# twosigma/Cook

Measured on AMD Instinct MI355X. Metric: match-cycles/sec at 1M pending x 50k offers, higher is better.
Workload: dtype f64

## Files before the change

cook_amd/csrc/classfit_asm.hpp:

```cpp
#pragma once
#if CF_SLOTS_N == 12
#define CF_O_CTRL "13728"
#define CF_O_CTRL4 "13732"
#define CF_O_ARR "15280"
#define CF_O_CLS32 "9504"
#define CF_SLOT_SHIFT "9"
#define CF_SLOT_N "12"
#define CF_ROW_END "3072"
#elif CF_SLOTS_N == 24
#define CF_O_CTRL "16800"
#define CF_O_CTRL4 "16804"
#define CF_O_ARR "18352"
#define CF_O_CLS32 "12576"
#define CF_SLOT_SHIFT "10"
#define CF_SLOT_N "24"
#define CF_ROW_END "6144"
#else
#error "CF_SLOTS_N: 12 or 24"
#endif
#ifndef CF_ASM_WAIT_READS
#define CF_ASM_WAIT_READS "30"
#endif
#ifdef CF_DELAY_D
#define CF_ASM_DELAY_D "s_sleep 6\n\t"
#else
#define CF_ASM_DELAY_D
#endif
#define CF_ASM_DECIDER_RUN \
   \
  "v_lshl_add_u32 v114, v65, 3, s56\n\t" \
  "ds_read_b64 v[114:115], v114\n\t" \
  "s_ff1_i32_b64 s44, s[42:43]\n\t" \
  "s_lshl_b32 s45, s44, 12\n\t" \
  "s_add_u32 s45, s45, s59\n\t" \
  "s_lshl_b32 s47, s57, 8\n\t" \
  "s_or_b32 s47, s47, s44\n\t" \
  "s_mov_b32 s41, 1\n\t"  \
   \
  "0:\n\t" \
  "v_readlane_b32 s60, v80, s44\n\t" \
  "v_readlane_b32 s61, v81, s44\n\t" \
  "v_readlane_b32 s62, v82, s44\n\t" \
  "s_and_b32 s63, s62, 0xffff00ff\n\t"  \
  "s_cmp_lg_u32 s63, 0\n\t" \
  "s_cbranch_scc1 9f\n\t" \
                                                                                           \
  "v_mov_b32_e32 v88, s47\n\t"                                                                                                          \
  "v_add_u32_e32 v100, s46, v83\n\t"                                                                                                    \
  "s_mov_b64 exec, 1\n\t"                                                                                                               \
  "ds_write_b32 v87, v88 offset:" CF_O_CTRL4 "\n\t"                                                                                              \
  "s_mov_b64 exec, -1\n\t"                                                                                                              \
  "s_mov_b32 s82, " CF_ASM_WAIT_READS "\n\t"              \
  "1:\n\t"                                                                                                                              \
  "ds_read_b32 v92, v100\n\t"                                                                                                           \
  "ds_read_b64 v[94:95], v100 offset:8\n\t"                                                                                             \
  "ds_read_b128 v[96:99], v100 offset:16\n\t"                                                                                           \
  "ds_read_b32 v93, v100\n\t"                                                                                                           \
                                        \
  "v_subrev_u32_e32 v101, s60, v71\n\t"                                                                                                 \
  "v_subrev_u32_e32 v102, s61, v72\n\t"                                                                                                 \
  "v_cvt_f64_u32_e32 v[104:105], v101\n\t"                                                                                              \
  "v_cvt_f64_u32_e32 v[106:107], v102\n\t"                                                                                              \
  "v_mul_f64 v[104:105], v[104:105], v[66:67]\n\t"                                                                                      \
  "v_mul_f64 v[106:107], v[106:107], v[68:69]\n\t"                                                                                      \
  "v_add_f64 v[104:105], v[104:105], v[106:107]\n\t"                                                                                    \
  "v_add_f64 v[104:105], -v[104:105], 1.0\n\t"                                                                                          \
  "v_cmp_le_u32_e64 s[64:65], s60, v71\n\t"                                                                                             \
  "v_cmp_le_u32_e64 s[66:67], s61, v72\n\t"                                                                                             \
  "v_cmp_ne_u32_e64 s[68:69], 0, v64\n\t"                                                                                               \
  "s_and_b64 s[64:65], s[64:65], s[66:67]\n\t"                                                                                          \
  "s_and_b64 s[64:65], s[64:65], s[68:69]\n\t"                                                                                          \
  "s_waitcnt lgkmcnt(0)\n\t"                                                                                                            \
        \
  "s_bfe_u32 s63, s62, 0x4000c\n\t"                                                                                                     \
  "s_cmp_eq_u32 s63, 0\n\t"                                                                                                             \
  "s_cbranch_scc1 3f\n\t"                                                                                                               \
  "v_readlane_b32 s66, v85, s44\n\t"                                                                                                    \
  "v_readlane_b32 s67, v86, s44\n\t"                                                                                                    \
  "s_cmp_lt_u32 s63, 1\n\t"                                                                                                           \
  "s_cbranch_scc1 3f\n\t"                                                                                                               \
  "s_bfe_u32 s72, s66, 0x100000\n\t"                                                                      \
  "s_lshr_b32 s73, s72, 8\n\t"                                                                                                          \
  "s_lshl_b32 s73, s73, 3\n\t"                                                                                                          \
  "s_and_b32 s72, s72, 0xff\n\t"                                                                                                        \
  "v_lshrrev_b64 v[108:109], s73, v[114:115]\n\t"                                                                                       \
  "v_and_b32_e32 v108, 0xff, v108\n\t"                                                                                                  \
  "v_cmp_eq_u32_e64 s[74:75], s72, v108\n\t"                                                                                            \
  "s_and_b64 s[64:65], s[64:65], s[74:75]\n\t"                                                                                          \
  "s_cmp_lt_u32 s63, 2\n\t"                                                                                                           \
  "s_cbranch_scc1 3f\n\t"                                                                                                               \
  "s_bfe_u32 s72, s66, 0x100010\n\t"                                                                      \
  "s_lshr_b32 s73, s72, 8\n\t"                                                                                                          \
  "s_lshl_b32 s73, s73, 3\n\t"                                                                                                          \
  "s_and_b32 s72, s72, 0xff\n\t"                                                                                                        \
  "v_lshrrev_b64 v[108:109], s73, v[114:115]\n\t"                                                                                       \
  "v_and_b32_e32 v108, 0xff, v108\n\t"                                                                                                  \
  "v_cmp_eq_u32_e64 s[74:75], s72, v108\n\t"                                                                                            \
  "s_and_b64 s[64:65], s[64:65], s[74:75]\n\t"                                                                                          \
  "s_cmp_lt_u32 s63, 3\n\t"                                                                                                           \
  "s_cbranch_scc1 3f\n\t"                                                                                                               \
  "s_bfe_u32 s72, s67, 0x100000\n\t"                                                                      \
  "s_lshr_b32 s73, s72, 8\n\t"                                                                                                          \
  "s_lshl_b32 s73, s73, 3\n\t"                                                                                                          \
  "s_and_b32 s72, s72, 0xff\n\t"                                                                                                        \
  "v_lshrrev_b64 v[108:109], s73, v[114:115]\n\t"                                                                                       \
  "v_and_b32_e32 v108, 0xff, v108\n\t"                                                                                                  \
  "v_cmp_eq_u32_e64 s[74:75], s72, v108\n\t"                                                                                            \
  "s_and_b64 s[64:65], s[64:65], s[74:75]\n\t"                                                                                          \
  "s_cmp_lt_u32 s63, 4\n\t"                                                                                                           \
  "s_cbranch_scc1 3f\n\t"                                                                                                               \
  "s_bfe_u32 s72, s67, 0x100010\n\t"                                                                      \
  "s_lshr_b32 s73, s72, 8\n\t"                                                                                                          \
  "s_lshl_b32 s73, s73, 3\n\t"                                                                                                          \
  "s_and_b32 s72, s72, 0xff\n\t"                                                                                                        \
  "v_lshrrev_b64 v[108:109], s73, v[114:115]\n\t"                                                                                       \
  "v_and_b32_e32 v108, 0xff, v108\n\t"                                                                                                  \
  "v_cmp_eq_u32_e64 s[74:75], s72, v108\n\t"                                                                                            \
  "s_and_b64 s[64:65], s[64:65], s[74:75]\n\t"                                                                                          \
  "3:\n\t"                                                                                                                              \
   \
  "v_and_b32_e32 v108, 0xffffff00, v92\n\t"                                                                                             \
  "v_cmp_eq_u32_e64 s[70:71], s45, v108\n\t"                                                                                            \
  "v_cmp_eq_u32_e64 s[72:73], v92, v93\n\t"                                                                                             \
  "v_sub_u32_e32 v108, v73, v92\n\t"                                                                                                    \
  "v_and_b32_e32 v108, 0xff, v108\n\t"                                                                                                  \
  "v_cmp_gt_u32_e64 s[74:75], 3, v108\n\t"                                                                                              \
  "v_and_b32_e32 v109, 0xffff, v94\n\t"                                                                                                 \
  "v_cmp_ne_u32_e64 s[76:77], v109, v74\n\t"                                                                                            \
  "v_cmp_ne_u32_e64 s[78:79], v109, v75\n\t"                                                                                            \
  "v_cmp_gt_i32_e64 s[80:81], 0, v95\n\t"                                                                                               \
  "s_and_b64 s[74:75], s[74:75], s[76:77]\n\t"                                                                                          \
  "s_and_b64 s[74:75], s[74:75], s[78:79]\n\t"                                                                                          \
  "s_or_b64 s[74:75], s[74:75], s[80:81]\n\t"                                                                                           \
  "s_and_b64 s[72:73], s[70:71], s[72:73]\n\t"                                          \
  "s_and_b64 s[70:71], s[72:73], s[74:75]\n\t"                                                                                            \
  "s_andn2_b64 s[76:77], s[52:53], s[70:71]\n\t"                                                                     \
  "s_cmp_eq_u64 s[76:77], 0\n\t"                                                                                                          \
  "s_cbranch_scc1 2f\n\t"                                                                                                                 \
   \
   \
  "s_and_b64 s[78:79], s[76:77], s[72:73]\n\t"                                                                                            \
  "s_cmp_eq_u64 s[78:79], 0\n\t"                                                                                                          \
  "s_cbranch_scc1 4f\n\t"                                                                                                                 \
  "v_and_b32_e32 v109, 0x3fff, v95\n\t"                                                                                                   \
  "s_and_b64 s[72:73], s[64:65], s[54:55]\n\t"                                                   \
  "10:\n\t"                                                                                                                               \
  "s_ff1_i32_b64 s83, s[78:79]\n\t"                                                                                                       \
  "v_readlane_b32 s63, v109, s83\n\t"                                                                                                     \
  "s_bitset0_b64 s[78:79], s83\n\t"                                                                                                       \
  "v_cmp_eq_u32_e64 vcc, s63, v65\n\t"                                                                                                    \
  "s_and_b64 vcc, vcc, s[72:73]\n\t"                                                                                                      \
  "s_cmp_eq_u64 vcc, 0\n\t"                                                                                                               \
  "s_cbranch_scc1 11f\n\t"                                                                                                                \
  "s_bitset1_b64 s[80:81], s83\n\t"                                                                                                       \
  "s_bitset0_b64 s[76:77], s83\n\t"                                                                                                       \
  "11:\n\t"                                                                                                                               \
  "s_cmp_lg_u64 s[78:79], 0\n\t"                                                                                                          \
  "s_cbranch_scc1 10b\n\t"                                                                                                                \
  "s_cmp_eq_u64 s[76:77], 0\n\t"                                                                                                          \
  "s_cbranch_scc1 2f\n\t"                                                                                                                 \
  "4:\n\t"                                                                                                                                \
  "s_sub_u32 s82, s82, 1\n\t"      \
  "s_cmp_eq_u32 s82, 0\n\t"                                                                                                             \
  "s_cbranch_scc1 9f\n\t"                                                                                                               \
  "s_sleep 1\n\t"                                                                                                                       \
  "s_branch 1b\n\t"                                                                                                                     \
  "2:\n\t"                                                                                                                              \
  "s_andn2_b64 s[74:75], s[52:53], s[80:81]\n\t"                                                                        \
  "s_or_b64 s[64:65], s[64:65], s[74:75]\n\t"                                                          \
  "v_cndmask_b32_e64 v110, v98, v104, s[54:55]\n\t"                                                                                     \
  "v_cndmask_b32_e64 v111, v99, v105, s[54:55]\n\t"                                                                                     \
  "v_cndmask_b32_e64 v110, 0, v110, s[64:65]\n\t"                                                                                       \
  "v_cndmask_b32_e64 v111, 0, v111, s[64:65]\n\t"                                                                                       \
  "v_cvt_f32_f64_e32 v112, v[110:111]\n\t" \
   \
   \
   \
  "s_mov_b64 s[84:85], s[42:43]\n\t" \
  "v_mov_b32_e32 v113, v112\n\t" \
  "s_bitset0_b64 s[84:85], s44\n\t" \
  "s_add_u32 s46, s46, 256\n\t" \
  "v_max_f32_dpp v113, v113, v113 quad_perm:[1,0,3,2] row_mask:0xf bank_mask:0xf\n\t" \
  "s_ff1_i32_b64 s86, s[84:85]\n\t" \
  "s_add_u32 s62, s57, 1\n\t" \
  "v_max_f32_dpp v113, v113, v113 quad_perm:[2,3,0,1] row_mask:0xf bank_mask:0xf\n\t" \
  "s_cmp_eq_u32 s46, " CF_ROW_END "\n\t" \
  "s_cselect_b32 s46, 0, s46\n\t" \
  "v_max_f32_dpp v113, v113, v113 row_half_mirror row_mask:0xf bank_mask:0xf\n\t" \
  "s_lshl_b32 s62, s62, 8\n\t" \
  "s_or_b32 s47, s62, s86\n\t" \
  "v_max_f32_dpp v113, v113, v113 row_mirror row_mask:0xf bank_mask:0xf\n\t" \
  "s_lshl_b32 s63, s86, 12\n\t" \
  "s_add_u32 s45, s59, s63\n\t" \
  "v_max_f32_dpp v113, v113, v113 row_bcast:15 row_mask:0xa bank_mask:0xf\n\t" \
  "v_add_f32_e32 v108, 0x35000000, v112\n\t" \
  "v_and_b32_e32 v109, 0x40000000, v95\n\t" \
  "v_max_f32_dpp v113, v113, v113 row_bcast:31 row_mask:0xc bank_mask:0xf\n\t" \
  "v_cmp_ne_u32_e64 s[70:71], 0, v109\n\t" \
  "s_nop 0\n\t" \
  "v_readlane_b32 s63, v113, 63\n\t" \
  "s_cmp_eq_u32 s63, 0\n\t" \
  "s_cbranch_scc1 8f\n\t"  \
  "v_cmp_eq_f32_e64 s[78:79], s63, v112\n\t" \
  "v_cmp_le_f32_e64 s[76:77], s63, v108\n\t"  \
  "s_and_b64 s[76:77], s[76:77], s[64:65]\n\t"                                      \
  "s_bcnt1_i32_b64 s62, s[76:77]\n\t"                                                                                                   \
  "s_cmp_gt_u32 s62, 1\n\t"                                                                                                             \
  "s_cbranch_scc1 9f\n\t"                                                                                                               \
  "s_and_b64 s[70:71], s[70:71], s[76:77]\n\t"                                                                                          \
  "s_and_b64 s[70:71], s[70:71], s[74:75]\n\t"                       \
  "s_cmp_lg_u64 s[70:71], 0\n\t"                                                                                                        \
  "s_cbranch_scc1 9f\n\t"                                                                                                               \
  "s_ff1_i32_b64 s82, s[78:79]\n\t"                                                                                                     \
  "s_cmp_lt_u32 s82, 58\n\t"                                                                                                            \
  "s_cbranch_scc0 5f\n\t"                                                                                                               \
                                                                                                         \
  "v_readlane_b32 s64, v71, s82\n\t"                                                                                                    \
  "v_readlane_b32 s65, v72, s82\n\t"                                                                                                    \
  "v_readlane_b32 s66, v65, s82\n\t"                                                                                                    \
  "s_sub_u32 s67, s64, s60\n\t"                                                                                                         \
  "s_sub_u32 s70, s65, s61\n\t"                                                                                                         \
  "v_cmp_eq_u32_e64 vcc, s82, v84\n\t"                                                                                                  \
  "v_mov_b32_e32 v88, s67\n\t"                                                                                                          \
  "v_mov_b32_e32 v89, s70\n\t"                                                                                                          \
  "s_cmp_lt_u32 s67, s49\n\t" \
  "s_cselect_b32 s71, 1, 0\n\t" \
  "s_cmp_lt_u32 s70, s50\n\t" \
  "s_cselect_b32 s71, 1, s71\n\t" \
  "v_cndmask_b32_e32 v71, v71, v88, vcc\n\t"                                                                                            \
  "v_cndmask_b32_e32 v72, v72, v89, vcc\n\t"                                                                                            \
  "s_cmp_lg_u32 s71, 0\n\t"                                                                                                             \
  "s_cselect_b64 s[62:63], vcc, 0\n\t"                             \
  "s_mov_b32 s72, s44\n\t"                                                                                                              \
  "s_mov_b32 s73, 0\n\t"                                                                                                                \
  "v_cndmask_b32_e64 v64, v64, 0, s[62:63]\n\t"                                                                                         \
  "s_branch 7f\n\t"                                                                                                                     \
        \
  "5:\n\t"                                                                                                                              \
  "v_readlane_b32 s64, v96, s82\n\t"                                                                                                    \
  "v_readlane_b32 s65, v97, s82\n\t"                                                                                                    \
  "v_readlane_b32 s76, v95, s82\n\t"                                                                                                    \
  "v_readlane_b32 s77, v94, s82\n\t"                                                                                                    \
  "v_readlane_b32 s78, v73, s82\n\t"                                                                                                    \
  "s_sub_u32 s67, s64, s60\n\t"                                                                                                         \
  "s_sub_u32 s70, s65, s61\n\t"                                                                                                         \
  "s_and_b32 s66, s76, 0x3fff\n\t"                                                                                                      \
  "s_bfe_u32 s79, s76, 0x80010\n\t"                                                                                                     \
  "s_and_b32 s73, s77, 0xffff\n\t"                                                                                                      \
  "s_lshr_b32 s81, s77, 16\n\t"                                                                                                         \
  "s_sub_u32 s80, s82, 57\n\t"                                                                                                          \
  "s_cmp_lt_u32 s67, s49\n\t" \
  "s_cselect_b32 s71, 1, 0\n\t" \
  "s_cmp_lt_u32 s70, s50\n\t" \
  "s_cselect_b32 s71, 1, s71\n\t" \
  "s_bcnt1_i32_b64 s62, s[68:69]\n\t"                                                                                                   \
  "s_cmp_lg_u32 s71, 0\n\t"                                                                                                             \
  "s_cbranch_scc1 6f\n\t"                                                                                                               \
  "s_cmp_ge_u32 s62, " CF_ASM_EPOCH_LIVE "\n\t"                                                                                          \
  "s_cbranch_scc1 9f\n\t"                                  \
  "6:\n\t"                                                                                                                              \
  "s_lshl_b32 s62, s73, 3\n\t" \
  "s_lshl_b32 s63, s80, 2\n\t" \
  "s_add_u32 s78, s78, 1\n\t" \
  "v_mov_b32_e32 v88, 0\n\t" \
  "v_mov_b32_e32 v89, 0\n\t" \
  "v_add_u32_e32 v90, s62, v87\n\t" \
  "v_add_u32_e32 v91, s63, v87\n\t" \
  "v_mov_b32_e32 v100, s78\n\t"                                                                                                         \
  "s_mov_b64 exec, 1\n\t"                                                                                                               \
  "ds_write_b64 v90, v[88:89] offset:" CF_O_ARR "\n\t"                                                                                         \
  "ds_write_b32 v91, v100 offset:" CF_O_CTRL4 "\n\t"                                                                                             \
  "s_mov_b64 exec, -1\n\t"                                                                                                              \
  "v_cmp_eq_u32_e64 vcc, s82, v84\n\t"                                                                                                  \
  "v_mov_b32_e32 v101, s73\n\t" \
  "s_lshl_b32 s62, s80, 8\n\t" \
  "v_cndmask_b32_e32 v75, v75, v74, vcc\n\t" \
  "v_cndmask_b32_e32 v74, v74, v101, vcc\n\t" \
  "v_cndmask_b32_e32 v73, v73, v100, vcc\n\t" \
  "s_lshl_b32 s63, s81, 12\n\t"                                                                                                         \
  "s_or_b32 s72, s44, s62\n\t"                                                                                                          \
  "s_or_b32 s72, s72, s63\n\t"                                                                                                          \
  "s_cmp_lg_u32 s71, 0\n\t"                                                                                                             \
  "s_cbranch_scc1 7f\n\t"                                                                              \
  "s_mul_i32 s62, s79, 56\n\t" \
  "v_add_u32_e32 v90, s62, v87\n\t" \
  "ds_read_b128 v[116:119], v90 offset:" CF_O_CLS32 "\n\t"  \
  "v_mov_b32_e32 v88, s66\n\t" \
  "v_lshl_add_u32 v102, v88, 3, s56\n\t"   \
  "ds_read_b64 v[102:103], v102\n\t"                                                                                        \
  "s_andn2_b64 s[62:63], s[54:55], s[68:69]\n\t"                                                                                        \
  "s_ff1_i32_b64 s83, s[62:63]\n\t"                                                                                                     \
  "v_cmp_eq_u32_e64 vcc, s83, v84\n\t"                                                                                                  \
  "v_mov_b32_e32 v89, s79\n\t"                                                                                                          \
  "v_mov_b32_e32 v91, s67\n\t"                                                                                                          \
  "v_mov_b32_e32 v101, s70\n\t"                                                                                                         \
  "v_cndmask_b32_e64 v64, v64, 1, vcc\n\t"                                                                                              \
  "v_cndmask_b32_e32 v65, v65, v88, vcc\n\t"                                                                                            \
  "v_cndmask_b32_e32 v70, v70, v89, vcc\n\t"                                                                                            \
  "v_cndmask_b32_e32 v71, v71, v91, vcc\n\t"                                                                                            \
  "v_cndmask_b32_e32 v72, v72, v101, vcc\n\t"                                                                                           \
  "s_waitcnt lgkmcnt(0)\n\t"                                                                                                            \
  "v_cndmask_b32_e32 v66, v66, v116, vcc\n\t"                                                                                           \
  "v_cndmask_b32_e32 v67, v67, v117, vcc\n\t"                                                                                           \
  "v_cndmask_b32_e32 v68, v68, v118, vcc\n\t"                                                                                           \
  "v_cndmask_b32_e32 v69, v69, v119, vcc\n\t"  \
  "v_cndmask_b32_e32 v114, v114, v102, vcc\n\t" \
  "v_cndmask_b32_e32 v115, v115, v103, vcc\n\t"                                                                                           \
   \
  "7:\n\t"                                                                                                                              \
  "v_cmp_eq_u32_e64 vcc, s44, v84\n\t"                                                                                                  \
  "v_mov_b32_e32 v88, s66\n\t"                                                                                                          \
  "v_cmp_lt_u32_e64 s[62:63], s67, v80\n\t"                                                                                             \
  "v_cmp_lt_u32_e64 s[76:77], s70, v81\n\t"                                                                                             \
  "v_cndmask_b32_e32 v76, v76, v88, vcc\n\t"                                                                                            \
  "s_or_b64 s[62:63], s[62:63], s[76:77]\n\t"                                                                                           \
  "s_lshl_b64 s[76:77], -2, s44\n\t"                                                                                                    \
  "s_and_b64 s[62:63], s[62:63], s[76:77]\n\t"                                                                                          \
  "s_or_b64 s[38:39], s[38:39], s[62:63]\n\t"                                                                                           \
  "s_min_u32 s37, s37, s67\n\t"                                                                                                         \
  "s_min_u32 s40, s40, s70\n\t"                                                                                                         \
  "s_add_u32 s36, s36, 1\n\t"                                                                                                           \
  "v_mov_b32_e32 v88, s72\n\t"                                                                                                          \
  "v_mov_b32_e32 v89, s73\n\t"                                                                                                          \
  "v_mov_b32_e32 v90, s64\n\t"                                                                                                          \
  "v_mov_b32_e32 v91, s65\n\t" \
  "s_mov_b64 exec, 1\n\t" \
  "ds_write_b128 v77, v[88:91]\n\t" \
  "s_mov_b64 exec, -1\n\t" \
  "v_add_u32_e32 v77, 32, v77\n\t"  \
   \
  "8:\n\t" \
  CF_ASM_DELAY_D \
  "s_mov_b64 s[42:43], s[84:85]\n\t" \
  "s_mov_b32 s44, s86\n\t" \
  "s_add_u32 s57, s57, 1\n\t" \
  "s_cmp_lg_u64 s[42:43], 0\n\t" \
  "s_cbranch_scc1 0b\n\t" \
  "s_mov_b32 s41, 0\n\t" \
  "9:\n\t" \
  "s_waitcnt lgkmcnt(0)\n\t"

#define CF_ASM_CLASS_STEP                                                                                                               \
  "v_mov_b32_e32 v80, s44\n\t"                                                                                                          \
  "s_lshl_b32 s60, s45, 2\n\t"                                                                                                          \
  "s_add_u32 s60, s60, s44\n\t"                                                                                                         \
  "v_mov_b32_e32 v81, s60\n\t"                                                                                                          \
  "ds_read_b64 v[82:83], v80 offset:" CF_O_CTRL "\n\t"                                                                     \
  "ds_read_b32 v84, v81 offset:" CF_O_CTRL4 "\n\t"                                                                   \
  "s_mov_b32 s41, 3\n\t"                                                                                                                \
  "s_waitcnt lgkmcnt(0)\n\t"                                                                                                            \
  "v_readfirstlane_b32 s61, v82\n\t"                                                                                                    \
  "v_readfirstlane_b32 s42, v83\n\t"                                                                                                    \
  "v_readfirstlane_b32 s43, v84\n\t"                                                                                                    \
  "s_cmp_lg_u32 s61, 0\n\t"                                                                                                             \
  "s_cbranch_scc1 9f\n\t"                                                                                                               \
  "s_cmp_lg_u32 s43, s40\n\t"                                                                                                           \
  "s_cbranch_scc1 9f\n\t"                                                                                                               \
  "s_mov_b32 s41, 2\n\t"                                                                                                                \
                                                                                                 \
  "1:\n\t"                                                                                                                              \
  "s_cmp_eq_u64 s[36:37], 0\n\t"                                                                                                        \
  "s_cbranch_scc1 9f\n\t"                                                                                                               \
  "s_cmp_eq_u32 s39, s56\n\t"                                                                                                           \
  "s_cbranch_scc1 2f\n\t"                                                                                                               \
  "s_add_u32 s62, s36, -1\n\t"                                                                                                          \
  "s_addc_u32 s63, s37, -1\n\t"                                                                                                         \
  "s_and_b64 s[36:37], s[36:37], s[62:63]\n\t"                                                                                          \
  "s_add_u32 s38, s38, 1\n\t"                                                                                                           \
  "s_add_u32 s39, s39, 1\n\t"                                                                                                           \
  "s_cmp_eq_u32 s39, s57\n\t"                                                                                                           \
  "s_cselect_b32 s39, 0, s39\n\t"                                                                                                       \
  "s_branch 1b\n\t"                                                                                                                     \
  "2:\n\t"                                                                                                                                \
  "s_lshr_b32 s60, s42, 8\n\t"                                                                                                            \
  "s_cmp_lt_u32 s38, s60\n\t"                                          \
  "s_cbranch_scc0 12f\n\t"                                                                                                                \
  "s_mov_b32 s41, 3\n\t"                                                                                                                  \
  "s_branch 9f\n\t"                                                                                                                       \
  "12:\n\t"                                                                                                                               \
  "s_add_u32 s60, s60, s59\n\t"                                                                                                         \
  "s_cmp_ge_u32 s38, s60\n\t"                                                                                                           \
  "s_cbranch_scc1 9f\n\t"                                                                             \
  "s_ff1_i32_b64 s64, s[36:37]\n\t"                                                                                                     \
  "v_readlane_b32 s65, v72, s64\n\t"                                                                                                    \
  "v_readlane_b32 s66, v73, s64\n\t"                                                                                                    \
  "v_readlane_b32 s67, v74, s64\n\t"                                                                                                    \
  "s_mov_b32 s41, 1\n\t"                                                                                                                \
  "s_lshr_b32 s60, s67, 12\n\t"                                                                                                         \
  "s_cmp_lg_u32 s60, 0\n\t"                                                                                                             \
  "s_cbranch_scc1 9f\n\t"                                                                                \
  "s_and_b32 s60, s67, 0xff\n\t"                                                                                                        \
  "s_cmp_lg_u32 s60, s58\n\t"                                                                                                           \
  "s_cbranch_scc1 8f\n\t"                                                                                \
                                           \
  "s_bfe_u32 s60, s67, 0x30008\n\t"                                                                                                     \
  "s_bitcmp1_b32 s60, 0\n\t"                                                                                                            \
  "s_cselect_b64 vcc, -1, 0\n\t"                                                                                                        \
  "v_cndmask_b32_e32 v80, v64, v65, vcc\n\t"                                                                                            \
  "v_cndmask_b32_e32 v81, v66, v67, vcc\n\t"                                                                                            \
  "v_cndmask_b32_e32 v82, v68, v69, vcc\n\t"                                                                                            \
  "v_cndmask_b32_e32 v83, v70, v71, vcc\n\t"                                                                                            \
  "s_bitcmp1_b32 s60, 1\n\t"                                                                                                            \
  "s_cselect_b64 vcc, -1, 0\n\t"                                                                                                        \
  "v_cndmask_b32_e32 v80, v80, v81, vcc\n\t"                                                                                            \
  "v_cndmask_b32_e32 v82, v82, v83, vcc\n\t"                                                                                            \
  "s_bitcmp1_b32 s60, 2\n\t"                                                                                                            \
  "s_cselect_b64 vcc, -1, 0\n\t"                                                                                                        \
  "v_cndmask_b32_e32 v80, v80, v82, vcc\n\t"                                                                                            \
                                                                 \
  "s_mul_i32 s68, s38, 43\n\t"                                                                                                          \
  "s_lshr_b32 s68, s68, " CF_SLOT_SHIFT "\n\t"                                                                                                          \
  "s_mul_i32 s68, s68, " CF_SLOT_N "\n\t"                                                                                                          \
// ... 84 lines not shown
```

cook_amd/csrc/classfit_host.hpp:

```cpp

static int classfit_env() {
  static const int v = [] {
    const char* s = std::getenv("COOK_CLASSFIT");
    return s && (s[0] == '0' || s[0] == '1') ? s[0] - '0' : -1;
  }();
  return v;
}
static bool classfit_by_default(const cook_engine* e) {
  const int f = classfit_env();
  if (f >= 0) return f == 1;
  return g_engines_on_device[e->device & 63].load() >= 6;
}
static size_t cf_lds_bytes_host(unsigned NP, unsigned M, bool eq, unsigned G, unsigned S) {
  size_t n = sizeof(CfFixed) + (size_t)NP * 10u;
  n = (n + 7u) & ~(size_t)7u;
  if (eq) n += (size_t)M * 8u;
  n += ((size_t)G + 1u) * 2u + (size_t)G * 2u + (size_t)S * 2u;
  return n + 64u;
}
bool cf_setup(cook_engine* e, const MatchIn& in, const MatchIn* in_dev, const MatchState& st, const JobRec* jr, const JobCons* jcons, const OfferA* oa, const OfferB* ob,
              CfPoolCtx& ctx) {
  const unsigned K = in.K, M = in.M, G = in.G;
  e->cf_inelig = 0x10000u;
  if (K == 0 || M == 0 || M > CF_SORT_N || G > CF_MAXG || in.good_enough < 1.0 || in.has_x || in.reserved_bits || in.host_dup) return false;
  if (e->cf_max_host == 0xFFFFFFFFu || (size_t)e->cf_max_host > 8u * (size_t)M + 65536u) return false;
  CfBuf b{};
  b.ctl = e->cf_ctl.ensure(1);
  b.jr = jr, b.jcons = jcons, b.oa = oa, b.ob = ob;
  b.attr8 = e->cf_attr8.ensure(M);
  b.max_host = e->cf_max_host;
  b.h2o = e->cf_h2o.ensure((size_t)b.max_host + 1u);
  b.pos_fc = e->cf_pos[0].ensure(M), b.pos_fm = e->cf_pos[1].ensure(M), b.pos_cid = e->cf_pos[2].ensure(M);
  b.scr_fc = e->cf_scr[0].ensure(M), b.scr_fm = e->cf_scr[1].ensure(M), b.scr_cid = e->cf_scr[2].ensure(M);
  b.jobs = e->cf_jobs.ensure(K);
  b.gcount = e->cf_gcount.ensure(std::max(1u, G));
  b.gmem = e->cf_gmem.ensure((size_t)std::max(1u, G) * CF_GMEM);
  static_assert(sizeof(CfCtl) % 4 == 0, "cf_init clears the control block word by word");
  KM<cf_init, 256>(e, "cf_init", std::min(div_up(b.max_host + 1u, 1024u), 512u), b, b.max_host + 1u, std::max(1u, G));
  KM<cf_scan, 256>(e, "cf_scan", div_up(std::max(K, M), 256), in_dev, b, K, M);
  KM<cf_prepare, 1024>(e, "cf_prepare", 1u, in_dev, b, st.jmin, K, M, G, in.host_dup, in.reserved_bits ? 1u : 0u);
  KM<cf_pack_jobs, 256>(e, "cf_pack_jobs", div_up(K, 256), in_dev, b, K);
  static_assert(offsetof(CfCtl, t) <= 512, "the control block's head is read back through the 512-byte scratch");
  pinned_copy(e, e->h_scratch, b.ctl, offsetof(CfCtl, t), hipMemcpyDeviceToHost);
  sync(e);
  CfCtl hc;
  std::memcpy((void*)&hc, e->h_scratch, offsetof(CfCtl, t));
  e->cf_inelig = hc.inelig;
  if (hc.inelig) return false;
  const unsigned NP = (M + 63u) & ~63u;
  const unsigned S = hc.any_group ? e->cf_group_run_total + hc.n_grouped : 0u;
  if (cf_lds_bytes_host(NP, M, hc.any_eq != 0u, hc.any_group ? G : 0u, S) > CF_LDS_BYTES || S > 60000u) {
    e->cf_inelig = CF_X_SHAPE;
    return false;
  }
  ctx.in = in_dev;
  ctx.st = st;
  ctx.b = b;
  return true;
}
static void cf_prof_print(const uint32_t* q) {
#ifdef CF_PROF
  std::fprintf(stderr, "CFPROF (x16 shader cycles) decider: slow steps %u (candidates %u evaluation %u commit %u) plain steps %u in %u walk-total %u | class wave 1: poll %u answer %u answers %u idle %u idles %u | class wave 2: poll %u answer %u answers %u idle %u idles %u | walk ticks(100MHz) %u | batch boundaries: decider %u, batches without a walked job %u\n", q[27], q[24], q[25], q[26], q[28], q[29], q[31], q[32], q[33], q[35], q[36], q[37], q[40], q[41], q[43], q[44], q[45], q[CFS_TICKS_WALK], q[30], q[38]);
  std::fprintf(stderr, "CFPROF plain steps %u, C++ steps %u; steps that left the plain form: gpu kind %u, novel hosts %u, group %u, answer missing after the re-reads %u, guard band %u, epoch end %u\n", q[46], q[47], q[34] & 65535u, q[34] >> 16, q[39] & 65535u, q[39] >> 16, q[42] & 65535u, q[42] >> 16);
#else
  (void)q;
#endif
}
void cf_run(cook_engine* lead, cook_engine* const* es, unsigned n, hipStream_t stream) {
  cook_engine* e = lead;
  for (unsigned i0 = 0; i0 < n; i0 += (unsigned)CF_PACK) {
    const unsigned c = std::min<unsigned>(CF_PACK, n - i0);
    CfPack pk{};
    for (unsigned x = 0; x < (unsigned)CF_PACK; ++x) pk.c[x] = es[i0 + (x < c ? x : 0u)]->placement.walk;
    KLS("cf_walk", stream, cf_walk, c, CF_THREADS, pk);
  }
  for (unsigned i = 0; i < n; ++i) {
    const CfPoolCtx& c = es[i]->placement.walk;
    const unsigned G = es[i]->last_in.G;
    if (G) KLS("cf_group_chains", stream, cf_group_chains, div_up(G, 256), 256, c.b, c.st, G);
  }
  constexpr size_t SLOT = 16 + 48 * 4;
  if (!lead->h_cf) COOK_HIP(hipHostMalloc((void**)&lead->h_cf, 64 * SLOT, hipHostMallocDefault));
  for (unsigned i = 0; i < n; ++i) {
    char* slot = lead->h_cf + i * SLOT;
    COOK_HIP(hipMemcpyAsync(slot, es[i]->placement.walk.st.summary, 16, hipMemcpyDeviceToHost, stream));
    COOK_HIP(hipMemcpyAsync(slot + 16, es[i]->placement.walk.b.ctl->stats, 48 * 4, hipMemcpyDeviceToHost, stream));
  }
  COOK_HIP(hipStreamSynchronize(stream));
  for (unsigned i = 0; i < n; ++i) {
    cook_engine* x = es[i];
    const unsigned* sum = (const unsigned*)(lead->h_cf + i * SLOT);
    if (sum[3] == 0xDEADu) lead->fail(COOK_E_STATE, "cf_walk: the pool's tables do not fit the workgroup's LDS (the host's check let it through)");
    std::memcpy(x->cf_stats, lead->h_cf + i * SLOT + 16, 48 * 4);
    cf_prof_print(x->cf_stats);
    WinCtl c{};
    c.matched = sum[0], c.head_matched = sum[1], c.rounds = sum[2], c.head = x->last_in.K, c.visited_sum = x->cf_stats[CFS_WALKED];
    c.t_seq = x->cf_stats[CFS_TICKS_TOTAL], c.t_setup = x->cf_stats[CFS_TICKS_PROLOGUE];
    x->placement_complete(3, c);
  }
}
```

cook_amd/csrc/classfit_walk.hpp:

```cpp
#pragma once
#if defined(CF_PROF) && !defined(CF_STATS)
#define CF_STATS 1
#endif
#ifdef CF_STATS
#define CF_STAT(x) x
#define CF_TICKS() cook_ticks()
#else
#define CF_STAT(x) ((void)0)
#define CF_TICKS() 0ull
#endif
#ifdef CF_PROF
#define CF_PROF_T(x) const unsigned long long x = __builtin_readcyclecounter()
#define CF_PROF_ADD(i, d) prof[i] += (unsigned long long)(d)
#define CF_PROF_WHY(n) why = why == 3u ? (n) : why
#define CF_PROF_LEAVE() (why < 4u ? leave_a += 1ull << (16u * why) : leave_b += 1ull << (16u * (why - 4u)))
#else
#define CF_PROF_T(x) ((void)0)
#define CF_PROF_ADD(i, d) ((void)0)
#define CF_PROF_WHY(n) ((void)0)
#define CF_PROF_LEAVE() ((void)0)
#endif

#ifndef CF_AHEAD
#define CF_AHEAD 10
// ... 446 lines not shown
    if (64u + lane < K) nxt = b.jobs[64u + lane];
#pragma unroll
    for (unsigned i = 0; i < CF_PRE; ++i) {
      pre[i] = nxt;
      if (64u * (i + 2u) + lane < K) pre[i] = b.jobs[64u * (i + 2u) + lane];
    }
  }
  if (is_decider) cook_set_prio_high();
  const unsigned long long t_loop = cook_ticks();
  __syncthreads();
  const bool isov = lane < CF_OVL;
  const unsigned clw = isov ? 0u : lane - CF_OVL + 1u;

  for (unsigned base = 0; base < K;) {
    const unsigned bn = cf_min(64u, K - base);
    const unsigned slot = (base >> 6) & 1u;
    const unsigned long long walkmask = wave_uniform_u64((unsigned long long)S.misc[CFX_WALK_LO] | (unsigned long long)S.misc[CFX_WALK_HI] << 32);
    const unsigned nw = (unsigned)__popcll(walkmask);
    st_walked += nw;
    if (!is_books) {
      const CfJob j = S.ring[slot * 64u + (lane < bn ? lane : 0u)];
      const bool in = lane < bn;
      jc = in ? j.c : 0u, jm = in ? j.m : 0u, jmeta = in ? j.meta : CF_KIND_NONE, jgrp = j.grp, jeq0 = j.eq[0], jeq1 = j.eq[1], jnov0 = j.nov[0], jnov1 = j.nov[1];
    }
    res = -1;
    if (is_decider) b1m = __ballot(!(jc <= minfc_all && jm <= minfm_all));
    unsigned logn = 0;
    unsigned long long todo = walkmask;
    unsigned cur_ord = 0;
    unsigned ph = 0;
    bool batch_done = nw == 0u;
    auto decider_books = [&](unsigned n_placed) {
      if (lane < bn) st.job_to_offer[base + lane] = res;
      const unsigned long long mm = __ballot(res >= 0);
      if (base == 0u) head = (unsigned)(mm & 1ull);
      const bool live = isov && o.valid != 0u;
      const unsigned nl = live ? cf_level_of(t, o.fc) : 0u;
#define CF_OV_T(i) unsigned v##i = nl > (unsigned)i ? o.fm + 1u : 0u;
      CF_FOR8(CF_OV_T)
#undef CF_OV_T
      wave_max8_u32(v0, v1, v2, v3, v4, v5, v6, v7);
      if (lane == 0) {
        S.misc[CFX_MATCH_LO] = (unsigned)mm, S.misc[CFX_MATCH_HI] = (unsigned)(mm >> 32), S.misc[CFX_B1_LO] = (unsigned)b1m, S.misc[CFX_B1_HI] = (unsigned)(b1m >> 32);
        S.misc[CFX_LOGN] = n_placed, S.misc[CFX_MINFC] = minfc_all, S.misc[CFX_MINFM] = minfm_all;
#define CF_OV_S(i) S.ovt[i] = v##i;
        CF_FOR8(CF_OV_S)
#undef CF_OV_S
      }
    };
    const unsigned long long tw0 = CF_TICKS();
    CF_PROF_T(cw0);
#ifdef CF_PROF
    if (is_decider && nw != 0u && bnd0 != 0ull) prof[6] += cw0 - bnd0, bnd0 = 0ull;
    if (is_class_wave && nw == 0u) prof[6] += 16ull;
#endif
    while (!batch_done) {
      unsigned md = 0;
      if (is_decider) {
#if COOK_HAS_ASM_WALK
        cf_u32x16 ST = {0u, 0u, 0u, 0u, 0u, 0u, 0u, 0u, 0u, 0u, 0u, 0u, 0u, 0u, 0u, 0u};
        const unsigned a_board = wave_uniform_u32(cook_lds_off(S.board)), a_log = wave_uniform_u32(cook_lds_off(S.log));
        cf_u32x8 JB = {jc, jm, jmeta, a_board + clw * (unsigned)sizeof(CfEnt), lane, jeq0, jeq1, a_board};
        const unsigned long long rel0 = cook_ballot(!isov & ((my_kinds & 1u) != 0u)), ovm = cf_below(CF_OVL);
        auto st_pack = [&] {
          const unsigned long long hc = (unsigned long long)__double_as_longlong(o.hTc), hm = (unsigned long long)__double_as_longlong(o.hTm);
          ST[0] = o.valid, ST[1] = o.id, ST[2] = (unsigned)hc, ST[3] = (unsigned)(hc >> 32), ST[4] = (unsigned)hm, ST[5] = (unsigned)(hm >> 32), ST[6] = o.cls, ST[7] = o.fc, ST[8] = o.fm,
          ST[9] = nrm, ST[10] = rm1, ST[11] = rm2, ST[12] = (unsigned)res, ST[13] = a_log + logn * (unsigned)sizeof(CfLog);
        };
        auto st_unpack = [&] {
          o.valid = ST[0], o.id = ST[1], o.hTc = __longlong_as_double((long long)((unsigned long long)ST[3] << 32 | ST[2])),
          o.hTm = __longlong_as_double((long long)((unsigned long long)ST[5] << 32 | ST[4])), o.cls = ST[6], o.fc = ST[7], o.fm = ST[8], nrm = ST[9], rm1 = ST[10], rm2 = ST[11],
          res = (int)ST[12];
        };
#endif
        while (md == 0u) {
          todo = wave_uniform_u64(todo), cur_ord = wave_uniform_u32(cur_ord), logn = wave_uniform_u32(logn), matched = wave_uniform_u32(matched), gen = wave_uniform_u32(gen);
          minfc_all = wave_uniform_u32(minfc_all), minfm_all = wave_uniform_u32(minfm_all), b1m = wave_uniform_u64(b1m);
#if COOK_HAS_ASM_WALK
          if (todo != 0ull) {
            st_pack();
            CF_PROF_T(f0);
#define CF_U(x) wave_uniform_u32((unsigned)(x))
            cf_u32x8 SC = {CF_U(matched), CF_U(minfc_all), CF_U(b1m), CF_U(b1m >> 32), CF_U(minfm_all), 1u, CF_U(todo), CF_U(todo >> 32)};
            cf_u32x8 AR = {0u, 0u, CF_U(cf_slot(cur_ord) * 8u * (unsigned)sizeof(CfEnt)), 0u, 0u, CF_U(cmin), CF_U(mmin), a_board};
            cf_u32x8 MK = {CF_U(rel0), CF_U(rel0 >> 32), CF_U(ovm), CF_U(ovm >> 32), CF_U(cook_lds_off(S.attr8)), CF_U(cur_ord), 0u, CF_U(base << 12 | (gen & 15u) << 8)};
            asm volatile(CF_ASM_DECIDER_RUN
                         : "+{v[64:79]}"(ST), "+{s[36:43]}"(SC), "+{s[44:51]}"(AR), "+{s[52:59]}"(MK)
                         : "{v[80:87]}"(JB)
                         : "v88", "v89", "v90", "v91", "v92", "v93", "v94", "v95", "v96", "v97", "v98", "v99", "v100", "v101", "v102", "v103", "v104", "v105", "v106", "v107", "v108",
                           "v109", "v110", "v111", "v112", "v113", "v114", "v115", "v116", "v117", "v118", "v119", "s60", "s61", "s62", "s63", "s64", "s65", "s66", "s67", "s68", "s69",
                           "s70", "s71", "s72", "s73", "s74", "s75", "s76", "s77", "s78", "s79", "s80", "s81", "s82", "s83", "s84", "s85", "s86", "vcc", "scc", "memory");
            matched = CF_U(SC[0]), minfc_all = CF_U(SC[1]), minfm_all = CF_U(SC[4]);
            b1m = wave_uniform_u64((unsigned long long)SC[3] << 32 | SC[2]);
            todo = wave_uniform_u64((unsigned long long)SC[7] << 32 | SC[6]);
            logn = (CF_U(ST[13]) - a_log) / (unsigned)sizeof(CfLog);
            CF_PROF_ADD(4, CF_U(MK[5]) - cur_ord);
            cur_ord = CF_U(MK[5]);
#undef CF_U
            CF_PROF_T(f1);
            CF_PROF_ADD(5, f1 - f0);
            WAIT_LDS();
            st_unpack();
          }
#endif
          if (todo == 0ull) {
#ifdef CF_PROF
            bnd0 = __builtin_readcyclecounter();
#endif
            decider_books(logn);
            md = CFM_BATCH_END;
            st_lane0_b32(&S.ctrl[0], md);
            break;
          }
          CF_PROF_T(p0);
          const unsigned s = (unsigned)__ffsll(todo) - 1u;
          const unsigned ord = cur_ord;
          st_lane0_b32(&S.ctrl[1], s | ord << 8);
          const unsigned Jc = (unsigned)wave_read_lane((int)jc, (int)s), Jm = (unsigned)wave_read_lane((int)jm, (int)s), meta = (unsigned)wave_read_lane((int)jmeta, (int)s);
          const unsigned kind = meta & 255u;
          const unsigned want = (base + s) << 12 | (gen & 15u) << 8;
#ifdef CF_PROF
          unsigned why = kind != 0u ? 0u : ((meta >> 16) & 15u) ? 1u : ((meta >> 20) & 1u) ? 2u : 3u;
#endif
          const CfEnt* e = &S.board[cf_slot(ord) * 8u + clw];
          const bool relevant = !isov && kind < 32u && ((my_kinds >> (kind & 31u)) & 1u);
          unsigned cpos, ccid, cfc, cfm;
          double cfa;
          bool acc;
          bool ok_ov = isov & (o.valid != 0u) & (kind == 0u) & (o.fc >= Jc) & (o.fm >= Jm);
          if (meta >> 12) {
            const CfJobU J = job_of(s);
            ok_ov = ok_ov & cf_cons_ok(S, J, o.id, ok_ov);
          }
          for (;;) {
            const unsigned t1 = ld_wg(&e->tag);
            COMPILER_FENCE();
            cpos = e->pos, ccid = e->cid, cfc = e->fc, cfm = e->fm, cfa = e->fa;
            COMPILER_FENCE();
            const unsigned t2 = ld_wg(&e->tag);
            const unsigned behind = (nrm - t1) & 255u, p = cpos & 0xFFFFu;
            const bool ours = (t1 == t2) & ((t1 & ~255u) == want);
            acc = ours & (((ccid & CF_ENT_NONE) != 0u) | ((behind <= 2u) & (p != rm1) & (p != rm2)));
            if (cook_ballot(relevant & !acc) == 0ull) break;
            for (unsigned long long rq = cook_ballot(relevant & !acc & ours); rq != 0ull; rq &= rq - 1ull) {
              const unsigned L = (unsigned)__ffsll(rq) - 1u;
              const unsigned xid = (unsigned)wave_read_lane((int)(ccid & CF_IDMASK), (int)L);
              if (cook_ballot(ok_ov & (o.id == xid)) != 0ull && lane == L) acc = true, ccid = CF_ENT_NONE;
            }
            if (cook_ballot(relevant & !acc) == 0ull) break;
            CF_STAT(++st_spins);
            SPIN_PAUSE_NEAR();
          }
          CF_PROF_T(p1);
          CF_PROF_ADD(0, p1 - p0);
          const unsigned vfc = isov ? o.fc : cfc, vfm = isov ? o.fm : cfm, vid = isov ? o.id : (ccid & CF_IDMASK);
          const bool vvalid = isov ? (o.valid != 0u && kind == 0u) : (relevant && !(ccid & CF_ENT_NONE));
          const bool room = vvalid & (vfc >= Jc) & (vfm >= Jm);
          const bool ok = isov ? ok_ov : room;
          double fov = 1.0 - ((double)(vfc - Jc) * o.hTc + (double)(vfm - Jm) * o.hTm);
          OPAQUE_V(fov);
          const double fa = ok ? (isov ? fov : cfa) : 0.0;
          const float ff = (float)fa;
          const float mx = wave_max_f32(ff);
          const unsigned long long eqm = cook_ballot(ok & (ff == mx)), nearm = cook_ballot(ok & (ff >= mx - CF_BAND32)),
                                   ambm = cook_ballot(ok & !isov & ((ccid & CF_ENT_AMB) != 0u) & (ff >= mx - CF_BAND32));
          CF_PROF_T(p2);
          CF_PROF_ADD(1, p2 - p1);
          CF_PROF_ADD(3, 1);
          if (!(mx > 0.0f)) {
            CF_PROF_LEAVE();
            todo &= todo - 1ull, ++cur_ord;
            continue;
          }
          unsigned l0 = (unsigned)__ffsll(eqm) - 1u;
          if ((nearm & (nearm - 1ull)) != 0ull || ambm != 0ull) {
            CF_PROF_WHY(4u);
            const unsigned long long mxb = wave_max_u64((unsigned long long)__double_as_longlong(fa));
            const double f0 = __longlong_as_double((long long)mxb);
            l0 = (unsigned)__ffsll(__ballot(ok && (unsigned long long)__double_as_longlong(fa) == mxb)) - 1u;
            const unsigned long long near = __ballot(ok && fa >= f0 - CF_BAND);
            const bool amb = (near & (near - 1ull)) != 0ull || (__ballot(ok && !isov && (ccid & CF_ENT_AMB) && fa >= f0 - CF_BAND) != 0ull);
            if (amb) {
              md = CFM_EXACT;
              if (lane == 0) S.misc[CFX_EX_LANE] = s, S.misc[CFX_FMAX_LO] = (unsigned)mxb, S.misc[CFX_FMAX_HI] = (unsigned)(mxb >> 32), st_wg(&S.ctrl[0], md);
              CF_PROF_LEAVE();
              break;
            }
          }
          todo &= todo - 1ull, ++cur_ord;
          const unsigned ofc = (unsigned)wave_read_lane((int)vfc, (int)l0), ofm = (unsigned)wave_read_lane((int)vfm, (int)l0), id = (unsigned)wave_read_lane((int)vid, (int)l0);
          const unsigned nfc = ofc - Jc, nfm = ofm - Jm;
          const bool dead = nfc < cmin || nfm < mmin;
          const bool from_ov = l0 < CF_OVL;
          ++matched;
          res = lane == s ? (int)id : res;
          b1m |= cook_ballot((jc > nfc) | (jm > nfm)) & ~cf_below(s) & ~(1ull << s);
          minfc_all = cf_min(minfc_all, nfc), minfm_all = cf_min(minfm_all, nfm);
          unsigned lpos = 0, linfo = s;
          if (from_ov) {
            CF_STAT(++st_ovwin);
            const bool me = lane == l0;
            o.fc = me ? nfc : o.fc, o.fm = me ? nfm : o.fm, o.valid = (me && dead) ? 0u : o.valid;
            if (dead) CF_STAT(++st_dead);
          } else {
            const bool gpu_place = kind != 0u;
// ... 683 lines not shown
```

Before: 23.34.

## Handle novel-host and small-group constraints inside the asm decider fast path

Steps whose jobs carry novel-host lists (up to four hosts) or a group constraint were previously sent out of the hand-written assembly fast path into the slower C++ path. The assembly now evaluates these itself: it builds an exclusion mask from the novel-host IDs, reads the group's host list from LDS when it has at most 16 entries, and on commit appends the chosen host to the group list. The intent is to keep more steps on the fast path. In exchange the asm block becomes more complex, adds extra LDS reads and writes per constrained step, and depends on the group bookkeeping staying consistent with the C++ path.

New measurement: 23.39, median of 6. About the same (+0.2%).

```diff
diff --git a/cook_amd/csrc/classfit_asm.hpp b/cook_amd/csrc/classfit_asm.hpp
--- a/cook_amd/csrc/classfit_asm.hpp
+++ b/cook_amd/csrc/classfit_asm.hpp
@@ -21,6 +21,8 @@
 #ifndef CF_ASM_WAIT_READS
 #define CF_ASM_WAIT_READS "30"
 #endif
+#define CF_ASM_GROUP_MAX 16
+#define CF_ASM_GROUP_B "16"
 #ifdef CF_DELAY_D
 #define CF_ASM_DELAY_D "s_sleep 6\n\t"
 #else
@@ -40,10 +42,11 @@
   "0:\n\t" \
   "v_readlane_b32 s60, v80, s44\n\t" \
   "v_readlane_b32 s61, v81, s44\n\t" \
-  "v_readlane_b32 s62, v82, s44\n\t" \
-  "s_and_b32 s63, s62, 0xffff00ff\n\t"  \
+  "v_readlane_b32 s87, v82, s44\n\t" \
+  "s_and_b32 s63, s87, 0xfffff0ff\n\t"  \
   "s_cmp_lg_u32 s63, 0\n\t" \
-  "s_cbranch_scc1 9f\n\t" \
+  "s_cbranch_scc1 20f\n\t" \
+  "21:\n\t" \
                                                                                            \
   "v_mov_b32_e32 v88, s47\n\t"                                                                                                          \
   "v_add_u32_e32 v100, s46, v83\n\t"                                                                                                    \
@@ -72,7 +75,10 @@
   "s_and_b64 s[64:65], s[64:65], s[68:69]\n\t"                                                                                          \
   "s_waitcnt lgkmcnt(0)\n\t"                                                                                                            \
         \
-  "s_bfe_u32 s63, s62, 0x4000c\n\t"                                                                                                     \
+  "s_cmp_lt_u32 s87, 0x1000\n\t"                           \
+  "s_cbranch_scc1 3f\n\t"                                                                                                               \
+  "s_and_b64 s[64:65], s[64:65], s[84:85]\n\t"  \
+  "s_bfe_u32 s63, s87, 0x4000c\n\t"                                                                                                     \
   "s_cmp_eq_u32 s63, 0\n\t"                                                                                                             \
   "s_cbranch_scc1 3f\n\t"                                                                                                               \
   "v_readlane_b32 s66, v85, s44\n\t"                                                                                                    \
@@ -235,6 +241,75 @@
   "s_mov_b32 s73, 0\n\t"                                                                                                                \
   "v_cndmask_b32_e64 v64, v64, 0, s[62:63]\n\t"                                                                                         \
   "s_branch 7f\n\t"                                                                                                                     \
+   \
+   \
+   \
+   \
+   \
+  "20:\n\t" \
+  "s_and_b32 s63, s87, 0xffe000ff\n\t" \
+  "s_cmp_lg_u32 s63, 0\n\t" \
+  "s_cbranch_scc1 9f\n\t" \
+  "s_mov_b64 s[84:85], -1\n\t" \
+  "s_bitcmp1_b32 s87, 20\n\t" \
+  "s_cbranch_scc0 22f\n\t" \
+  "v_readlane_b32 s66, %[grp], s44\n\t" \
+  "s_lshl_b32 s66, s66, 1\n\t" \
+  "s_add_u32 s67, s66, s48\n\t" \
+  "s_add_u32 s66, s66, s58\n\t" \
+  "v_mov_b32_e32 v116, s67\n\t" \
+  "v_mov_b32_e32 v118, s66\n\t" \
+  "ds_read_u16 v116, v116\n\t" \
+  "ds_read_u16 v117, v118\n\t" \
+  "22:\n\t" \
+  "s_bfe_u32 s63, s87, 0x40010\n\t" \
+  "s_cmp_eq_u32 s63, 0\n\t" \
+  "s_cbranch_scc1 23f\n\t" \
+  "v_readlane_b32 s66, %[nov0], s44\n\t" \
+  "v_readlane_b32 s67, %[nov1], s44\n\t" \
+  "s_and_b32 s72, s66, 0xffff\n\t" \
+  "v_cmp_ne_u32_e64 s[84:85], s72, v65\n\t" \
+  "s_cmp_lt_u32 s63, 2\n\t" \
+  "s_cbranch_scc1 23f\n\t" \
+  "s_lshr_b32 s72, s66, 16\n\t" \
+  "v_cmp_ne_u32_e64 s[74:75], s72, v65\n\t" \
+  "s_and_b64 s[84:85], s[84:85], s[74:75]\n\t" \
+  "s_cmp_lt_u32 s63, 3\n\t" \
+  "s_cbranch_scc1 23f\n\t" \
+  "s_and_b32 s72, s67, 0xffff\n\t" \
+  "v_cmp_ne_u32_e64 s[74:75], s72, v65\n\t" \
+  "s_and_b64 s[84:85], s[84:85], s[74:75]\n\t" \
+  "s_cmp_lt_u32 s63, 4\n\t" \
+  "s_cbranch_scc1 23f\n\t" \
+  "s_lshr_b32 s72, s67, 16\n\t" \
+  "v_cmp_ne_u32_e64 s[74:75], s72, v65\n\t" \
+  "s_and_b64 s[84:85], s[84:85], s[74:75]\n\t" \
+  "23:\n\t" \
+  "s_bitcmp1_b32 s87, 20\n\t" \
+  "s_cbranch_scc0 21b\n\t" \
+  "s_waitcnt lgkmcnt(0)\n\t" \
+  "v_readfirstlane_b32 s63, v117\n\t" \
+  "s_cmp_gt_u32 s63, " CF_ASM_GROUP_B "\n\t" \
+  "s_cbranch_scc1 9f\n\t" \
+  "v_add_u32_e32 v119, v116, v117\n\t" \
+  "v_add_u32_e32 v116, v116, v84\n\t" \
+  "v_add_u32_e32 v117, 1, v117\n\t" \
+  "v_lshl_add_u32 v119, v119, 1, %[gids]\n\t" \
+  "v_lshl_add_u32 v116, v116, 1, %[gids]\n\t" \
+  "s_bfm_b64 s[74:75], s63, 0\n\t" \
+  "s_mov_b64 exec, s[74:75]\n\t"  \
+  "ds_read_u16 v116, v116\n\t" \
+  "s_mov_b64 exec, -1\n\t" \
+  "s_mov_b32 s66, 0\n\t" \
+  "s_waitcnt lgkmcnt(0)\n\t" \
+  "24:\n\t" \
+  "s_cmp_ge_u32 s66, s63\n\t" \
+  "s_cbranch_scc1 21b\n\t" \
+  "v_readlane_b32 s72, v116, s66\n\t" \
+  "s_add_u32 s66, s66, 1\n\t" \
+  "v_cmp_ne_u32_e64 s[74:75], s72, v65\n\t" \
+  "s_and_b64 s[84:85], s[84:85], s[74:75]\n\t" \
+  "s_branch 24b\n\t" \
         \
   "5:\n\t"                                                                                                                              \
   "v_readlane_b32 s64, v96, s82\n\t"                                                                                                    \
@@ -284,7 +359,7 @@
   "s_cbranch_scc1 7f\n\t"                                                                              \
   "s_mul_i32 s62, s79, 56\n\t" \
   "v_add_u32_e32 v90, s62, v87\n\t" \
-  "ds_read_b128 v[116:119], v90 offset:" CF_O_CLS32 "\n\t"  \
+  "ds_read_b128 v[104:107], v90 offset:" CF_O_CLS32 "\n\t"  \
   "v_mov_b32_e32 v88, s66\n\t" \
   "v_lshl_add_u32 v102, v88, 3, s56\n\t"   \
   "ds_read_b64 v[102:103], v102\n\t"                                                                                        \
@@ -300,10 +375,10 @@
   "v_cndmask_b32_e32 v71, v71, v91, vcc\n\t"                                                                                            \
   "v_cndmask_b32_e32 v72, v72, v101, vcc\n\t"                                                                                           \
   "s_waitcnt lgkmcnt(0)\n\t"                                                                                                            \
-  "v_cndmask_b32_e32 v66, v66, v116, vcc\n\t"                                                                                           \
-  "v_cndmask_b32_e32 v67, v67, v117, vcc\n\t"                                                                                           \
-  "v_cndmask_b32_e32 v68, v68, v118, vcc\n\t"                                                                                           \
-  "v_cndmask_b32_e32 v69, v69, v119, vcc\n\t"  \
+  "v_cndmask_b32_e32 v66, v66, v104, vcc\n\t"                                                                                           \
+  "v_cndmask_b32_e32 v67, v67, v105, vcc\n\t"                                                                                           \
+  "v_cndmask_b32_e32 v68, v68, v106, vcc\n\t"                                                                                           \
+  "v_cndmask_b32_e32 v69, v69, v107, vcc\n\t"  \
   "v_cndmask_b32_e32 v114, v114, v102, vcc\n\t" \
   "v_cndmask_b32_e32 v115, v115, v103, vcc\n\t"                                                                                           \
    \
@@ -328,6 +403,15 @@
   "ds_write_b128 v77, v[88:91]\n\t" \
   "s_mov_b64 exec, -1\n\t" \
   "v_add_u32_e32 v77, 32, v77\n\t"  \
+   \
+   \
+  "s_bitcmp1_b32 s87, 20\n\t" \
+  "s_cbranch_scc0 8f\n\t" \
+  "v_mov_b32_e32 v88, s66\n\t" \
+  "s_mov_b64 exec, 1\n\t" \
+  "ds_write_b16 v119, v88\n\t" \
+  "ds_write_b16 v118, v117\n\t" \
+  "s_mov_b64 exec, -1\n\t" \
    \
   "8:\n\t" \
   CF_ASM_DELAY_D \
diff --git a/cook_amd/csrc/classfit_host.hpp b/cook_amd/csrc/classfit_host.hpp
--- a/cook_amd/csrc/classfit_host.hpp
+++ b/cook_amd/csrc/classfit_host.hpp
@@ -61,7 +61,7 @@
 static void cf_prof_print(const uint32_t* q) {
 #ifdef CF_PROF
   std::fprintf(stderr, "CFPROF (x16 shader cycles) decider: slow steps %u (candidates %u evaluation %u commit %u) plain steps %u in %u walk-total %u | class wave 1: poll %u answer %u answers %u idle %u idles %u | class wave 2: poll %u answer %u answers %u idle %u idles %u | walk ticks(100MHz) %u | batch boundaries: decider %u, batches without a walked job %u\n", q[27], q[24], q[25], q[26], q[28], q[29], q[31], q[32], q[33], q[35], q[36], q[37], q[40], q[41], q[43], q[44], q[45], q[CFS_TICKS_WALK], q[30], q[38]);
-  std::fprintf(stderr, "CFPROF plain steps %u, C++ steps %u; steps that left the plain form: gpu kind %u, novel hosts %u, group %u, answer missing after the re-reads %u, guard band %u, epoch end %u\n", q[46], q[47], q[34] & 65535u, q[34] >> 16, q[39] & 65535u, q[39] >> 16, q[42] & 65535u, q[42] >> 16);
+  std::fprintf(stderr, "CFPROF plain steps %u, C++ steps %u; steps that left the plain form: gpu kind %u, novel hosts %u, a group's list over the run's bound %u, answer missing after the re-reads %u, guard band %u, epoch end %u\n", q[46], q[47], q[34] & 65535u, q[34] >> 16, q[39] & 65535u, q[39] >> 16, q[42] & 65535u, q[42] >> 16);
 #else
   (void)q;
 #endif
diff --git a/cook_amd/csrc/classfit_walk.hpp b/cook_amd/csrc/classfit_walk.hpp
--- a/cook_amd/csrc/classfit_walk.hpp
+++ b/cook_amd/csrc/classfit_walk.hpp
@@ -552,14 +552,14 @@
             CF_PROF_T(f0);
 #define CF_U(x) wave_uniform_u32((unsigned)(x))
             cf_u32x8 SC = {CF_U(matched), CF_U(minfc_all), CF_U(b1m), CF_U(b1m >> 32), CF_U(minfm_all), 1u, CF_U(todo), CF_U(todo >> 32)};
-            cf_u32x8 AR = {0u, 0u, CF_U(cf_slot(cur_ord) * 8u * (unsigned)sizeof(CfEnt)), 0u, 0u, CF_U(cmin), CF_U(mmin), a_board};
-            cf_u32x8 MK = {CF_U(rel0), CF_U(rel0 >> 32), CF_U(ovm), CF_U(ovm >> 32), CF_U(cook_lds_off(S.attr8)), CF_U(cur_ord), 0u, CF_U(base << 12 | (gen & 15u) << 8)};
+            cf_u32x8 AR = {0u, 0u, CF_U(cf_slot(cur_ord) * 8u * (unsigned)sizeof(CfEnt)), 0u, CF_U(cook_lds_off(S.goff)), CF_U(cmin), CF_U(mmin), a_board};
+            cf_u32x8 MK = {CF_U(rel0), CF_U(rel0 >> 32), CF_U(ovm), CF_U(ovm >> 32), CF_U(cook_lds_off(S.attr8)), CF_U(cur_ord), CF_U(cook_lds_off(S.gcnt)), CF_U(base << 12 | (gen & 15u) << 8)};
             asm volatile(CF_ASM_DECIDER_RUN
                          : "+{v[64:79]}"(ST), "+{s[36:43]}"(SC), "+{s[44:51]}"(AR), "+{s[52:59]}"(MK)
-                         : "{v[80:87]}"(JB)
+                         : "{v[80:87]}"(JB), [grp] "v"(jgrp), [nov0] "v"(jnov0), [nov1] "v"(jnov1), [gids] "s"(CF_U(cook_lds_off(S.gids)))
                          : "v88", "v89", "v90", "v91", "v92", "v93", "v94", "v95", "v96", "v97", "v98", "v99", "v100", "v101", "v102", "v103", "v104", "v105", "v106", "v107", "v108",
                            "v109", "v110", "v111", "v112", "v113", "v114", "v115", "v116", "v117", "v118", "v119", "s60", "s61", "s62", "s63", "s64", "s65", "s66", "s67", "s68", "s69",
-                           "s70", "s71", "s72", "s73", "s74", "s75", "s76", "s77", "s78", "s79", "s80", "s81", "s82", "s83", "s84", "s85", "s86", "vcc", "scc", "memory");
+                           "s70", "s71", "s72", "s73", "s74", "s75", "s76", "s77", "s78", "s79", "s80", "s81", "s82", "s83", "s84", "s85", "s86", "s87", "vcc", "scc", "memory");
             matched = CF_U(SC[0]), minfc_all = CF_U(SC[1]), minfm_all = CF_U(SC[4]);
             b1m = wave_uniform_u64((unsigned long long)SC[3] << 32 | SC[2]);
             todo = wave_uniform_u64((unsigned long long)SC[7] << 32 | SC[6]);
@@ -590,7 +590,11 @@
           const unsigned kind = meta & 255u;
           const unsigned want = (base + s) << 12 | (gen & 15u) << 8;
 #ifdef CF_PROF
+#if COOK_HAS_ASM_WALK
+          unsigned why = kind != 0u ? 0u : (((meta >> 20) & 1u) && S.gcnt[(unsigned)wave_read_lane((int)jgrp, (int)s)] > (unsigned)CF_ASM_GROUP_MAX) ? 2u : 3u;
+#else
           unsigned why = kind != 0u ? 0u : ((meta >> 16) & 15u) ? 1u : ((meta >> 20) & 1u) ? 2u : 3u;
+#endif
 #endif
           const CfEnt* e = &S.board[cf_slot(ord) * 8u + clw];
           const bool relevant = !isov && kind < 32u && ((my_kinds >> (kind & 31u)) & 1u);
```
